# bharath5673/StrongSORT-YOLO

Hardware: NVIDIA B200
Metric: tracked frames/sec at 1080p, 100 dets/frame (higher is better)
Workload: dtype fp16 hi/lo operand pairs (~22-bit mantissa) with fp32 accumulate on tcgen05 (ReID convs, appearance cost) + fp32 (depthwise, decode, NMS) + f64 (Kalman, gating, IoU, LSAP)

## Files before the change

### strongsort-yolo_b200/csrc/reid_tc4.cu

```cuda
#include <cooperative_groups.h>

#include "ssb_common.cuh"
#include "tc_common.cuh"

namespace cg = cooperative_groups;

#ifndef SSB_DW_CHAINS
#define SSB_DW_CHAINS 3
#endif

namespace {

__host__ __device__ constexpr int cmax4(int a, int b) { return a > b ? a : b; }
__host__ __device__ constexpr int rup128_4(int a) { return (a + 127) / 128 * 128; }
__host__ __device__ constexpr int pow2cols(int c) { return c <= 32 ? 32 : c <= 64 ? 64 : c <= 128 ? 128 : c <= 256 ? 256 : 512; }

template <int CIN_, int MID_, int MIDP_, int COUT_, int H_, int W_, int R_, int NB_, bool DOWN_, int SEG_,
          int THREADS_, int MINB_, bool SPLIT_, bool PW_ = false>
struct B4 {
    static constexpr bool PW = PW_;
    static constexpr int CIN = CIN_, MID = MID_, MIDP = MIDP_, COUT = COUT_, H = H_, W = W_, R = R_, NB = NB_;
    static constexpr int SEG = SEG_, THREADS = THREADS_, MINB = MINB_;
    static constexpr bool DOWN = DOWN_, SPLIT = SPLIT_, EXCH = NB_ > 1;
    static constexpr int NWARPS = THREADS / 32, GROUPS = THREADS / 128;
    static constexpr int HW = H * W;
    static constexpr int NPX = R * W;
    static constexpr int NT = NPX / 128;
    static constexpr int MCH = MIDP / 8;
    static constexpr int CG = MID / 4;
    static constexpr int XL = W < 16 ? W : 16;
    static constexpr int CPW = 16 / XL;
    static constexpr int NCB = W / XL;
    static constexpr int NCGW = (CG / 2) / CPW;
    static constexpr int TPS = NCB * NCGW;
    static constexpr int PLANE_B = NPX * 16;
    static constexpr int MAP_HALF_B = MCH * PLANE_B, MAP_B = 2 * MAP_HALF_B;
    static constexpr int XCH = CIN / 8;
    static constexpr int XS_HALF_B = XCH * PLANE_B, XS_B = 2 * XS_HALF_B;
    static constexpr int TW = W + 2, TH = R + 2, TPX = TW * TH;
    static constexpr int T_B = CG * TPX * 16;
    static constexpr int A_B = rup128_4(cmax4(MAP_B + T_B, XS_B));
    static constexpr int LCN = 2 * MIDP;
    static constexpr int TM_C3 = NT * LCN, TM_COLS = TM_C3 + NT * COUT, TM_ALLOC = pow2cols(TM_COLS);
    static constexpr int C1W_B = CIN * MIDP * 4;
    static constexpr int DNW_HALF_B = DOWN ? CIN * COUT * 2 : 0, DNW_B = 2 * DNW_HALF_B;
    static constexpr int LCW_B = MIDP * MIDP * 4;
    static constexpr int WALL_B = C1W_B + DNW_B + 10 * LCW_B;
    static constexpr int PWW_HALF_B = COUT * COUT * 2, PWW_B = 2 * PWW_HALF_B;
    static constexpr int C3W_HALF_B = MIDP * COUT * 2, C3W_B = 2 * C3W_HALF_B;
    static constexpr int P_B1 = 0, P_LC = MIDP, P_B3 = P_LC + 100 * MIDP, P_GW1 = P_B3 + COUT;
    static constexpr int P_GB1 = P_GW1 + 2 * MIDP, P_GW2 = P_GB1 + 2, P_GB2 = P_GW2 + 2 * MIDP;
    static constexpr int NPAR = P_GB2 + MIDP;
    static constexpr int OFF_X1 = 0;
    static constexpr int OFF_A = OFF_X1 + MAP_B;
    static constexpr int OFF_W = OFF_A + A_B;
    static constexpr int OFF_C3 = OFF_W + rup128_4(WALL_B);
    static constexpr int OFF_PAR = OFF_C3 + C3W_B;
    static constexpr int OFF_GAP = OFF_PAR + rup128_4(NPAR * 4);
    static constexpr int OFF_MISC = OFF_GAP + 4 * NB * MIDP * 4;
    static constexpr int SCR_FLOATS = SEG * NCB * CG * 4;
    static constexpr int SMEM_B = OFF_MISC + 192 + (SCR_FLOATS + 2 * MIDP) * 4 + 64;
    static constexpr int SMEM_LIMIT = MINB >= 2 ? (232448 / MINB - 1024) : 232448;
    static_assert(NPX % 128 == 0, "band = whole M tiles");
    static_assert((W & (W - 1)) == 0, "W power of two");
    static_assert(NT <= 8, "per-tile barriers");
    static_assert(TM_ALLOC * MINB <= 512, "TMEM columns of the co-resident CTAs");
    static_assert(SMEM_B <= SMEM_LIMIT, "shared memory");
    static_assert(MIDP % 16 == 0 && COUT % 32 == 0 && CIN % 16 == 0 && MID % 4 == 0, "MMA shapes");
    static_assert(H % R == 0 && H / R == NB && NB <= 8, "bands / portable cluster size");
    static_assert(MID <= MIDP && COUT == 4 * MID && MIDP <= 32 && COUT * (MIDP / 8) <= THREADS, "OSBlock channel plan");
    static_assert(CG % 2 == 0 && (CG / 2) % CPW == 0 && W % XL == 0, "depthwise warp tasks");
    static_assert(SEG * TPS <= NWARPS, "depthwise warp tasks fit the CTA");
    static_assert(WALL_B + XS_B < (1 << 20), "mbarrier tx count");
    static_assert(!PW || (!DOWN && CIN == COUT && R % 2 == 0 && (PWW_B <= MAP_B || PWW_B <= WALL_B)), "fused transition");
    static constexpr int G_PAR = rup128_4(WALL_B);
    static constexpr int G_W3 = G_PAR + rup128_4(NPAR * 4);
    static constexpr int G_TOTAL = G_W3 + MIDP * COUT * 4;
};

__device__ __forceinline__ void split2(float a, float b, __half2 &h, __half2 &l) {
    h = __floats2half2_rn(a, b);
    const float2 hf = __half22float2(h);
    l = __floats2half2_rn(a - hf.x, b - hf.y);
}
__device__ __forceinline__ void split2p(float a, float b, __half2 &h, __half2 &l) {
    h = __floats2half2_rn(a, b);
    const float2 hf = __half22float2(h);
    unsigned long long v = ((unsigned long long)__float_as_uint(b) << 32) | __float_as_uint(a);
    const unsigned long long hv = ((unsigned long long)__float_as_uint(hf.y) << 32) | __float_as_uint(hf.x);
    asm("sub.rn.f32x2 %0, %0, %1;" : "+l"(v) : "l"(hv));
    l = __floats2half2_rn(__uint_as_float((uint32_t)v), __uint_as_float((uint32_t)(v >> 32)));
}
__device__ __forceinline__ void split1(float v, __half &h, __half &l) {
    h = __float2half_rn(v);
    l = __float2half_rn(v - __half2float(h));
}
__device__ __forceinline__ uint64_t dadv(uint64_t base, int units16) {
    return base + (uint64_t)(int64_t)units16;
}
__device__ __forceinline__ void mma3(uint32_t d, uint64_t ah, uint64_t al, uint64_t bh, uint64_t bl,
                                     uint32_t idesc, uint32_t acc) {
    tc::mma_f16_ss(d, ah, bh, idesc, acc);
    tc::mma_f16_ss(d, al, bh, idesc, 1);
    tc::mma_f16_ss(d, ah, bl, idesc, 1);
}
__device__ __forceinline__ void tmem_ld4_nw(uint32_t taddr, uint32_t *r) {
    asm volatile("tcgen05.ld.sync.aligned.32x32b.x4.b32 {%0, %1, %2, %3}, [%4];"
                 : "=r"(r[0]), "=r"(r[1]), "=r"(r[2]), "=r"(r[3])
                 : "r"(taddr)
                 : "memory");
}
__device__ __forceinline__ void tmem_ld8_nw(uint32_t taddr, uint32_t *r) {
    asm volatile("tcgen05.ld.sync.aligned.32x32b.x8.b32 {%0, %1, %2, %3, %4, %5, %6, %7}, [%8];"
                 : "=r"(r[0]), "=r"(r[1]), "=r"(r[2]), "=r"(r[3]), "=r"(r[4]), "=r"(r[5]), "=r"(r[6]), "=r"(r[7])
                 : "r"(taddr)
                 : "memory");
}
__device__ __forceinline__ void tmem_wait_ld() {
    asm volatile("tcgen05.wait::ld.sync.aligned;" ::: "memory");
}
__device__ __forceinline__ void cluster_arrive() { asm volatile("barrier.cluster.arrive.release.aligned;" ::: "memory"); }
__device__ __forceinline__ void cluster_wait() { asm volatile("barrier.cluster.wait.acquire.aligned;" ::: "memory"); }
__device__ __forceinline__ void cluster_arrive_relaxed() { asm volatile("barrier.cluster.arrive.relaxed.aligned;" ::: "memory"); }
__device__ __forceinline__ void st_cluster_f4(uint32_t cluster_addr, float a, float b, float c, float d) {
    asm volatile("st.shared::cluster.v4.f32 [%0], {%1, %2, %3, %4};" ::"r"(cluster_addr), "f"(a), "f"(b), "f"(c), "f"(d)
                 : "memory");
}
struct P4 { unsigned long long a, b; };
__device__ __forceinline__ P4 ldp4(const float4 *p) {
    const ulonglong2 v = *reinterpret_cast<const ulonglong2 *>(p);
    return P4{v.x, v.y};
}
__device__ __forceinline__ void fma4(P4 &o, const P4 &w, const P4 &v) {
    asm("fma.rn.f32x2 %0, %1, %2, %0;" : "+l"(o.a) : "l"(w.a), "l"(v.a));
    asm("fma.rn.f32x2 %0, %1, %2, %0;" : "+l"(o.b) : "l"(w.b), "l"(v.b));
}
__device__ __forceinline__ void mul4(P4 &o, const P4 &w, const P4 &v) {
    asm("mul.rn.f32x2 %0, %1, %2;" : "=l"(o.a) : "l"(w.a), "l"(v.a));
    asm("mul.rn.f32x2 %0, %1, %2;" : "=l"(o.b) : "l"(w.b), "l"(v.b));
}
__device__ __forceinline__ void add4(P4 &o, const P4 &v) {
    asm("add.rn.f32x2 %0, %0, %1;" : "+l"(o.a) : "l"(v.a));
    asm("add.rn.f32x2 %0, %0, %1;" : "+l"(o.b) : "l"(v.b));
}
__device__ __forceinline__ float p4x(const P4 &v) { return __uint_as_float((uint32_t)v.a); }
__device__ __forceinline__ float p4y(const P4 &v) { return __uint_as_float((uint32_t)(v.a >> 32)); }
__device__ __forceinline__ float p4z(const P4 &v) { return __uint_as_float((uint32_t)v.b); }
__device__ __forceinline__ float p4w(const P4 &v) { return __uint_as_float((uint32_t)(v.b >> 32)); }

__device__ __forceinline__ void unsplit8(const uint4 &h, const uint4 &l, float *out) {
    const __half2 *hh = reinterpret_cast<const __half2 *>(&h);
    const __half2 *ll = reinterpret_cast<const __half2 *>(&l);
#pragma unroll
    for (int j = 0; j < 4; j++) {
        const float2 a = __half22float2(hh[j]), b = __half22float2(ll[j]);
        out[2 * j] = a.x + b.x;
        out[2 * j + 1] = a.y + b.y;
    }
}

template <class C>
__global__ void __launch_bounds__(C::THREADS, C::MINB)
osblock4_kernel(const unsigned char *__restrict__ x, unsigned char *__restrict__ y,
                const unsigned char *__restrict__ wblob, int n_crops, int *__restrict__ status,
                long long *__restrict__ dbg, const unsigned char *__restrict__ pwblob) {
    extern __shared__ __align__(1024) unsigned char smem[];
    cg::cluster_group cluster = cg::this_cluster();
    const int tid = threadIdx.x, warp = tid >> 5, lane = tid & 31;
    const int quad = warp & 3, grp = warp >> 2;
    const int warp_u = __shfl_sync(0xffffffffu, warp, 0);
    const int crop = blockIdx.x / C::NB, band = blockIdx.x % C::NB;

    unsigned char *sX1 = smem + C::OFF_X1, *sP = smem + C::OFF_A;
    float4 *sT = reinterpret_cast<float4 *>(sP + C::MAP_B);
    unsigned char *sW = smem + C::OFF_W, *sC3 = smem + C::OFF_C3;
    float *sPar = reinterpret_cast<float *>(smem + C::OFF_PAR);
    float *sGap = reinterpret_cast<float *>(smem + C::OFF_GAP);
    uint64_t *bar_w = reinterpret_cast<uint64_t *>(smem + C::OFF_MISC);
    uint64_t *bar_c1 = bar_w + 1;
    uint64_t *bar_tile = bar_w + 3;
    uint64_t *bar_c3 = bar_w + 11;
    uint32_t *s_tmem = reinterpret_cast<uint32_t *>(bar_w + 16);
    float *s_scr = reinterpret_cast<float *>(smem + C::OFF_MISC + 192);

    if (warp == 0) tc::tmem_alloc(s_tmem, C::TM_ALLOC);
    if (tid == 0) {
        tc::mbar_init(bar_w, 1);
        tc::mbar_init(bar_c1, 1);
        for (int i = 0; i < 8; i++) tc::mbar_init(bar_tile + i, 1);
        tc::mbar_init(bar_c3, 1);
        tc::fence_mbar_init();
    }
    tc::fence_before_sync();
    __syncthreads();
    tc::fence_after_sync();
    const uint32_t tmem = *s_tmem;
    int dbg_n = 0;
    auto stamp = [&]() { if (dbg && blockIdx.x == 0 && tid == 0 && dbg_n < 63) dbg[1 + dbg_n++] = clock64(); };
#ifdef SSB_FINE_STAMPS
    int dbg_f = 0;
    auto fstamp = [&](int layer) {
        if (dbg && blockIdx.x == 0 && tid == 0 && (layer == 1 || layer == 2) && dbg_f < 40) { dbg[65 + dbg_f++] = clock64(); dbg[64] = dbg_f; }
    };
#else
    auto fstamp = [](int) {};
#endif
    stamp();
    bool ok = true;

    const unsigned char *xin = x + (size_t)crop * (4 * C::CIN * C::HW);
    constexpr int X_LO = 2 * C::CIN * C::HW;
    tc::pdl_launch_dependents();
    if (tid == 0) {
        constexpr int PAR_B = (C::NPAR * 4 + 15) / 16 * 16;
        tc::mbar_arrive_expect_tx(bar_w, C::WALL_B + C::XS_B + PAR_B);
        for (int o = 0; o < C::WALL_B; o += 32768) {
            const int nb = C::WALL_B - o < 32768 ? C::WALL_B - o : 32768;
            tc::bulk_g2s(sW + o, wblob + o, nb, bar_w);
        }
        tc::bulk_g2s(sPar, wblob + C::G_PAR, PAR_B, bar_w);
        tc::pdl_wait();
        for (int hl = 0; hl < 2; hl++)
            for (int ch = 0; ch < C::XCH; ch++)
                tc::bulk_g2s(sP + hl * C::XS_HALF_B + ch * C::PLANE_B,
                             xin + hl * X_LO + (size_t)ch * C::HW * 16 + (size_t)band * C::PLANE_B, C::PLANE_B, bar_w);
    }

    constexpr uint32_t IDESC_MID = tc::make_idesc_f16(128, C::MIDP);
    constexpr uint32_t IDESC_CAT = tc::make_idesc_f16(128, 2 * C::MIDP);
    constexpr uint32_t IDESC_OUT = tc::make_idesc_f16(128, C::COUT);
    const bool issuer = warp_u == (C::SEG * C::TPS < C::NWARPS ? C::SEG * C::TPS : 0);

    if (!tc::mbar_wait(bar_w, 0)) ok = false;
    tc::fence_after_sync();
    if (issuer) {
        if (tc::elect_one()) {
            const uint64_t ah0 = tc::make_smem_desc(tc::smem_u32(sP), C::PLANE_B, 128);
            const uint64_t al0 = dadv(ah0, C::XS_HALF_B / 16);
            const uint64_t bc0 = tc::make_smem_desc(tc::smem_u32(sW), 2 * C::MIDP * 16, 128);
#pragma unroll
            for (int t = 0; t < C::NT; t++) {
                const uint32_t d1 = tmem + t * C::LCN;
#pragma unroll
                for (int ks = 0; ks < C::CIN / 16; ks++) {
                    const int ka = t * 128 + ks * 2 * C::NPX;
                    tc::mma_f16_ss(d1, dadv(ah0, ka), dadv(bc0, ks * 4 * C::MIDP), IDESC_CAT, ks > 0);
                    tc::mma_f16_ss(d1, dadv(al0, ka), dadv(bc0, ks * 4 * C::MIDP), IDESC_MID, 1);
                }
                if (C::DOWN) {
                    const uint64_t dh0 = tc::make_smem_desc(tc::smem_u32(sW) + C::C1W_B, C::COUT * 16, 128);
                    const uint64_t dl0 = dadv(dh0, C::DNW_HALF_B / 16);
                    const uint32_t d2 = tmem + C::TM_C3 + t * C::COUT;
#pragma unroll
                    for (int ks = 0; ks < C::CIN / 16; ks++) {
                        const int ka = t * 128 + ks * 2 * C::NPX;
                        mma3(d2, dadv(ah0, ka), dadv(al0, ka), dadv(dh0, ks * 2 * C::COUT),
                             dadv(dl0, ks * 2 * C::COUT), IDESC_OUT, ks > 0);
                    }
                }
            }
            tc::mma_commit(bar_c1);
        }
        __syncwarp();
    }
    if (!tc::mbar_wait(bar_c1, 0)) ok = false;
    tc::fence_after_sync();
    stamp();

    for (int i = tid; i < (C::MAP_B + C::T_B) / 16; i += C::THREADS)
        reinterpret_cast<uint4 *>(sP)[i] = make_uint4(0u, 0u, 0u, 0u);
    {
        constexpr int NU1 = C::NT * C::MCH, UPT1 = (NU1 + C::GROUPS - 1) / C::GROUPS;
        uint32_t va[UPT1][8], vb[UPT1][8];
#pragma unroll
        for (int e = 0; e < UPT1; e++) {
            const int u = grp + e * C::GROUPS;
            if (u < NU1) {
                const int t = u / C::MCH, kc = u - t * C::MCH;
                const uint32_t ta = tmem + ((uint32_t)(quad * 32) << 16) + t * C::LCN + kc * 8;
                tmem_ld8_nw(ta, va[e]);
                tmem_ld8_nw(ta + C::MIDP, vb[e]);
            }
        }
        tmem_wait_ld();
#pragma unroll
        for (int e = 0; e < UPT1; e++) {
            const int u = grp + e * C::GROUPS;
            if (u < NU1) {
                const int t = u / C::MCH, kc = u - t * C::MCH;
                const int p = t * 128 + quad * 32 + lane;
                const float *bias = sPar + C::P_B1 + kc * 8;
                __align__(16) __half2 h[4];
                __align__(16) __half2 l[4];
#pragma unroll
                for (int j = 0; j < 8; j += 2) {
                    const float f0 = fmaxf(__uint_as_float(va[e][j]) + __uint_as_float(vb[e][j]) + bias[j], 0.f);
                    const float f1 = fmaxf(__uint_as_float(va[e][j + 1]) + __uint_as_float(vb[e][j + 1]) + bias[j + 1], 0.f);
                    split2(f0, f1, h[j >> 1], l[j >> 1]);
                }
                unsigned char *d_hi = sX1 + kc * C::PLANE_B + p * 16;
                *reinterpret_cast<uint4 *>(d_hi) = *reinterpret_cast<uint4 *>(h);
                *reinterpret_cast<uint4 *>(d_hi + C::MAP_HALF_B) = *reinterpret_cast<uint4 *>(l);
            }
        }
    }
    bool a_pending = false;
    if (C::EXCH) { cluster_arrive(); a_pending = true; }
    tc::fence_async_smem();
    tc::fence_before_sync();
    __syncthreads();
    tc::fence_after_sync();
    stamp();

    auto issue_pw = [&](const unsigned char *src, int layer, int t0, int t1) {
        const uint64_t ah0 = tc::make_smem_desc(tc::smem_u32(src), C::PLANE_B, 128);
        const uint64_t al0 = dadv(ah0, C::MAP_HALF_B / 16);
        const uint64_t b0 = tc::make_smem_desc(tc::smem_u32(sW) + C::C1W_B + C::DNW_B + layer * C::LCW_B,
                                               2 * C::MIDP * 16, 128);
#pragma unroll
        for (int t = 0; t < C::NT; t++) {
            if (t < t0 || t >= t1) continue;
            const uint32_t d = tmem + t * C::LCN;
            if (tc::elect_one()) {
#pragma unroll
                for (int ks = 0; ks < C::MIDP / 16; ks++) {
                    tc::mma_f16_ss(d, dadv(ah0, t * 128 + ks * 2 * C::NPX), dadv(b0, ks * 4 * C::MIDP), IDESC_CAT, ks > 0);
                    tc::mma_f16_ss(d, dadv(al0, t * 128 + ks * 2 * C::NPX), dadv(b0, ks * 4 * C::MIDP), IDESC_MID, 1);
                }
                tc::mma_commit(bar_tile + t);
            }
            __syncwarp();
        }
    };
    tc::pdl_wait();
    float w3r[8];
    {
        const float *w3 = reinterpret_cast<const float *>(wblob + C::G_W3);
        const int kc = tid / C::COUT, co = tid - kc * C::COUT;
#pragma unroll
        for (int j = 0; j < 8; j++) w3r[j] = tid < C::COUT * C::MCH ? w3[(kc * 8 + j) * C::COUT + co] : 0.f;
    }
    const int dw_par = lane & 1;
    const int dw_seg = warp / C::TPS, dw_cb = (warp % C::TPS) % C::NCB;
    const int dw_cg = (((warp % C::TPS) / C::NCB) * C::CPW + lane / (2 * C::XL)) * 2 + dw_par;
    const int dw_col = dw_cb * C::XL + (lane >> 1) % C::XL;
    const uint32_t sT_up = (C::EXCH && band > 0) ? tc::mapa_u32(sT, band - 1) : 0u;
    const uint32_t sT_dn = (C::EXCH && band < C::NB - 1) ? tc::mapa_u32(sT, band + 1) : 0u;
    int lc = 0;
    uint32_t tile_par = 0, c3_par = 0;
    bool c3_pending = false;
    if (issuer) issue_pw(sX1, 0, 0, C::NT);
    for (int s = 0; s < 4; s++) {
        for (int k = 0; k <= s; k++, lc++) {
            const bool last = (k == s);
            P4 wd[9], bs;
            {
                const float *wl = sPar + C::P_LC + lc * (10 * C::MIDP) + dw_cg * 4;
#pragma unroll
                for (int tap = 0; tap < 9; tap++) wd[tap] = ldp4(reinterpret_cast<const float4 *>(wl + tap * C::MIDP));
                bs = ldp4(reinterpret_cast<const float4 *>(wl + 9 * C::MIDP));
            }
            fstamp(lc);
            {
                constexpr int NU = C::NT * C::CG, UPT = (NU + C::GROUPS - 1) / C::GROUPS;
                uint32_t ra_[UPT][4], rb_[UPT][4];
#pragma unroll
                for (int i = 0; i < UPT; i++) {
                    const int u = grp + i * C::GROUPS;
                    if (u >= NU) continue;
                    const int t = u / C::CG, cgi = u - t * C::CG;
                    if (!tc::mbar_wait(bar_tile + t, tile_par)) ok = false;
                    tc::fence_after_sync();
                    const uint32_t ta = tmem + ((uint32_t)(quad * 32) << 16) + t * C::LCN + cgi * 4;
                    tmem_ld4_nw(ta, ra_[i]);
                    tmem_ld4_nw(ta + C::MIDP, rb_[i]);
                }
                tmem_wait_ld();
                fstamp(lc);
                if (a_pending) { cluster_wait(); a_pending = false; }
                fstamp(lc);
#pragma unroll
                for (int i = 0; i < UPT; i++) {
                    const int u = grp + i * C::GROUPS;
                    if (u >= NU) continue;
                    const int t = u / C::CG, cgi = u - t * C::CG;
                    const int p = t * 128 + quad * 32 + lane;
                    const int lr = p / C::W, col = p % C::W;
                    const float v0 = __uint_as_float(ra_[i][0]) + __uint_as_float(rb_[i][0]);
                    const float v1 = __uint_as_float(ra_[i][1]) + __uint_as_float(rb_[i][1]);
                    const float v2 = __uint_as_float(ra_[i][2]) + __uint_as_float(rb_[i][2]);
                    const float v3 = __uint_as_float(ra_[i][3]) + __uint_as_float(rb_[i][3]);
                    sT[cgi * C::TPX + (lr + 1) * C::TW + col + 1] = make_float4(v0, v1, v2, v3);
                    if (C::EXCH) {
                        if (lr == 0 && sT_up)
                            st_cluster_f4(sT_up + (uint32_t)(cgi * C::TPX + (C::R + 1) * C::TW + col + 1) * 16u, v0, v1, v2, v3);
                        if (lr == C::R - 1 && sT_dn)
                            st_cluster_f4(sT_dn + (uint32_t)(cgi * C::TPX + col + 1) * 16u, v0, v1, v2, v3);
                    }
                }
            }
            tile_par ^= 1;
            fstamp(lc);
            tc::fence_before_sync();
            if (C::EXCH) { cluster_arrive(); cluster_wait(); }
            else __syncthreads();
            tc::fence_after_sync();
            fstamp(lc);
            stamp();
            if (C::PW && lc == 9 && tid == 0) {
                unsigned char *dstw = C::PWW_B <= C::MAP_B ? sX1 : sW;
                tc::mbar_arrive_expect_tx(bar_w, C::PWW_B);
                for (int o = 0; o < C::PWW_B; o += 32768) {
                    const int nb = C::PWW_B - o < 32768 ? C::PWW_B - o : 32768;
                    tc::bulk_g2s(dstw + o, pwblob + o, nb, bar_w);
                }
            }
            if (last && s < 3 && issuer) issue_pw(sX1, lc + 1, 0, C::NT);
            if (k == 0 && c3_pending) {
                if (!tc::mbar_wait(bar_c3, c3_par)) ok = false;
                c3_par ^= 1;
                c3_pending = false;
                tc::fence_after_sync();
            }
            float4 gacc = make_float4(0.f, 0.f, 0.f, 0.f);
            auto dw_rows = [&](int ra, int rb) {
                if (rb <= ra) return;
                if (dw_seg >= C::SEG) return;
                const int r0 = ra + ((rb - ra) * dw_seg) / C::SEG, r1 = ra + ((rb - ra) * (dw_seg + 1)) / C::SEG;
                if (r0 >= r1) return;
                const float4 *Tp = sT + dw_cg * C::TPX + dw_col;
                unsigned char *dbase = sP + (dw_cg >> 1) * C::PLANE_B + dw_col * 16 + dw_par * 8;
                auto ldrow = [&](P4 *w, int trow) {
#pragma unroll
                    for (int j = 0; j < 3; j++) w[j] = ldp4(Tp + trow * C::TW + j);
                };
                auto dwrow = [&](int lr, const P4 *wa, const P4 *wb, const P4 *wc) {
#if SSB_DW_CHAINS == 3
                    P4 o = bs, o1, o2;
                    fma4(o, wd[0], wa[0]);
                    mul4(o1, wd[3], wb[0]);
                    mul4(o2, wd[6], wc[0]);
                    fma4(o, wd[1], wa[1]);
                    fma4(o1, wd[4], wb[1]);
                    fma4(o2, wd[7], wc[1]);
                    fma4(o, wd[2], wa[2]);
                    fma4(o1, wd[5], wb[2]);
                    fma4(o2, wd[8], wc[2]);
                    add4(o1, o2);
                    add4(o, o1);
#else
                    P4 o = bs;
#pragma unroll
                    for (int dx = 0; dx < 3; dx++) {
                        fma4(o, wd[dx], wa[dx]);
                        fma4(o, wd[3 + dx], wb[dx]);
                        fma4(o, wd[6 + dx], wc[dx]);
                    }
#endif
                    const float ox = fmaxf(p4x(o), 0.f), oy = fmaxf(p4y(o), 0.f);
                    const float oz = fmaxf(p4z(o), 0.f), ow = fmaxf(p4w(o), 0.f);
                    if (last) { gacc.x += ox; gacc.y += oy; gacc.z += oz; gacc.w += ow; }
                    __half2 h[2], l[2];
                    split2p(ox, oy, h[0], l[0]);
                    split2p(oz, ow, h[1], l[1]);
                    unsigned char *d = dbase + lr * (C::W * 16);
                    *reinterpret_cast<uint2 *>(d) = make_uint2(*reinterpret_cast<uint32_t *>(&h[0]), *reinterpret_cast<uint32_t *>(&h[1]));
                    *reinterpret_cast<uint2 *>(d + C::MAP_HALF_B) =
                        make_uint2(*reinterpret_cast<uint32_t *>(&l[0]), *reinterpret_cast<uint32_t *>(&l[1]));
                };
                P4 w0[3], w1[3], w2[3];
                ldrow(w0, r0);
                ldrow(w1, r0 + 1);
                for (int lr = r0; lr < r1; lr += 3) {
                    ldrow(w2, lr + 2);
                    dwrow(lr, w0, w1, w2);
                    if (lr + 1 < r1) {
                        ldrow(w0, lr + 3);
                        dwrow(lr + 1, w1, w2, w0);
                    }
                    if (lr + 2 < r1) {
                        ldrow(w1, lr + 4);
                        dwrow(lr + 2, w2, w0, w1);
                    }
                }
            };
            auto publish = [&]() {
                tc::fence_async_smem();
                tc::fence_before_sync();
                __syncthreads();
                tc::fence_after_sync();
            };
            if (!last) {
                if (C::SPLIT && C::NT >= 2) {
                    constexpr int TH_ = C::NT / 2, HR = TH_ * 128 / C::W;
                    dw_rows(0, HR);
                    publish();
                    if (issuer) issue_pw(sP, lc + 1, 0, TH_);
                    dw_rows(HR, C::R);
                    if (C::EXCH) { cluster_arrive_relaxed(); a_pending = true; }
                    publish();
                    if (issuer) issue_pw(sP, lc + 1, TH_, C::NT);
                } else {
                    dw_rows(0, C::R);
                    fstamp(lc);
                    if (C::EXCH) { cluster_arrive_relaxed(); a_pending = true; }
                    publish();
                    fstamp(lc);
                    if (issuer) issue_pw(sP, lc + 1, 0, C::NT);
                    fstamp(lc);
                }
                stamp();
                continue;
            }
            dw_rows(0, C::R);
            fstamp(lc);
            {
#pragma unroll
                for (int off = C::XL; off >= 2; off >>= 1) {
                    gacc.x += __shfl_xor_sync(0xffffffffu, gacc.x, off);
                    gacc.y += __shfl_xor_sync(0xffffffffu, gacc.y, off);
                    gacc.z += __shfl_xor_sync(0xffffffffu, gacc.z, off);
                    gacc.w += __shfl_xor_sync(0xffffffffu, gacc.w, off);
                }
                if (dw_seg < C::SEG && ((lane >> 1) % C::XL) == 0)
                    *reinterpret_cast<float4 *>(s_scr + ((dw_seg * C::NCB + dw_cb) * C::CG + dw_cg) * 4) = gacc;
            }
            publish();
            fstamp(lc);
            stamp();
            if (warp == 0 && lane < C::MIDP) {
                float tot = 0.f;
                if (lane < C::MID)
                    for (int g = 0; g < C::SEG * C::NCB; g++) tot += s_scr[(g * C::CG + (lane >> 2)) * 4 + (lane & 3)];
                float *slot = sGap + (s * C::NB + band) * C::MIDP + lane;
                if (C::NB > 1) {
#pragma unroll
                    for (int b = 0; b < C::NB; b++) tc::st_cluster_f32(tc::mapa_u32(slot, b), tot);
                } else {
                    *slot = tot;
                }
            }
            fstamp(lc);
            if (C::NB > 1) cluster.sync(); else __syncthreads();
            fstamp(lc);
            if (warp * 32 < C::COUT * C::MCH) {
                float tot = 0.f;
                if (lane < C::MIDP)
                    for (int b = 0; b < C::NB; b++) tot += sGap[(s * C::NB + b) * C::MIDP + lane];
                const float m = tot / (float)(C::H * C::W);
                float h0 = lane < C::MIDP ? m * sPar[C::P_GW1 + lane * 2 + 0] : 0.f;
                float h1 = lane < C::MIDP ? m * sPar[C::P_GW1 + lane * 2 + 1] : 0.f;
#pragma unroll
                for (int off = 16; off >= 1; off >>= 1) {
                    h0 += __shfl_xor_sync(0xffffffffu, h0, off);
                    h1 += __shfl_xor_sync(0xffffffffu, h1, off);
                }
                h0 = fmaxf(h0 + sPar[C::P_GB1 + 0], 0.f);
                h1 = fmaxf(h1 + sPar[C::P_GB1 + 1], 0.f);
                float gate = 0.f;
                if (lane < C::MIDP) {
                    float g = sPar[C::P_GB2 + lane];
                    g = fmaf(h0, sPar[C::P_GW2 + lane], g);
                    g = fmaf(h1, sPar[C::P_GW2 + C::MIDP + lane], g);
                    gate = 1.f / (1.f + expf(-g));
                }
                const int u = tid;
                const int kc = u / C::COUT;
                __align__(16) __half h[8];
                __align__(16) __half l[8];
#pragma unroll
                for (int j = 0; j < 8; j++) {
                    const float gk = __shfl_sync(0xffffffffu, gate, (kc * 8 + j) & 31);
                    split1(w3r[j] * gk, h[j], l[j]);
                }
                if (u < C::COUT * C::MCH) {
                    *reinterpret_cast<uint4 *>(sC3 + (size_t)u * 16) = *reinterpret_cast<uint4 *>(h);
                    *reinterpret_cast<uint4 *>(sC3 + C::C3W_HALF_B + (size_t)u * 16) = *reinterpret_cast<uint4 *>(l);
                }
            }
            fstamp(lc);
            tc::fence_async_smem();
            tc::fence_before_sync();
            __syncthreads();
            tc::fence_after_sync();
            if (issuer) {
                const uint64_t ah0 = tc::make_smem_desc(tc::smem_u32(sP), C::PLANE_B, 128);
                const uint64_t al0 = dadv(ah0, C::MAP_HALF_B / 16);
                const uint64_t bh0 = tc::make_smem_desc(tc::smem_u32(sC3), C::COUT * 16, 128);
                const uint64_t bl0 = dadv(bh0, C::C3W_HALF_B / 16);
                const uint32_t acc0 = (C::DOWN || s > 0) ? 1u : 0u;
                if (tc::elect_one()) {
#pragma unroll
                    for (int i = 0; i < C::NT; i++) {
                        const uint32_t d = tmem + C::TM_C3 + i * C::COUT;
#pragma unroll
                        for (int ks = 0; ks < C::MIDP / 16; ks++) {
                            const int ka = i * 128 + ks * 2 * C::NPX, kb = ks * 2 * C::COUT;
                            mma3(d, dadv(ah0, ka), dadv(al0, ka), dadv(bh0, kb), dadv(bl0, kb), IDESC_OUT,
                                 ks > 0 ? 1u : acc0);
                        }
                    }
                    tc::mma_commit(bar_c3);
                }
                __syncwarp();
            }
            c3_pending = true;
            stamp();
        }
    }

    unsigned char *yout = y + (size_t)crop * (4 * C::COUT * C::HW);
    constexpr int Y_LO = 2 * C::COUT * C::HW;
    constexpr int CCH = C::COUT / 32;
    constexpr int NUE = C::NT * CCH, UE = (NUE + C::GROUPS - 1) / C::GROUPS;
    constexpr bool PREF = !C::DOWN && UE <= 2;
    uint4 xh[PREF ? UE : 1][4], xl[PREF ? UE : 1][4];
    auto load_res = [&](int u, uint4 *h, uint4 *l) {
        const int i = u / CCH, c0 = (u - i * CCH) * 32;
        const size_t gp = (size_t)band * C::NPX + i * 128 + quad * 32 + lane;
#pragma unroll
        for (int j = 0; j < 4; j++) {
            const unsigned char *src = xin + (size_t)(c0 / 8 + j) * C::HW * 16 + gp * 16;
            h[j] = *reinterpret_cast<const uint4 *>(src);
            l[j] = *reinterpret_cast<const uint4 *>(src + X_LO);
        }
    };
    if (PREF) {
#pragma unroll
        for (int e = 0; e < UE; e++) {
            const int u = grp + e * C::GROUPS;
            if (u < NUE) load_res(u, xh[PREF ? e : 0], xl[PREF ? e : 0]);
        }
    }
    if (c3_pending) {
        if (!tc::mbar_wait(bar_c3, c3_par)) ok = false;
        c3_par ^= 1;
    }
    tc::fence_after_sync();
#pragma unroll
    for (int e = 0; e < UE; e++) {
        const int u = grp + e * C::GROUPS;
        if (u >= NUE) continue;
        const int i = u / CCH, c0 = (u - i * CCH) * 32;
        const size_t gp = (size_t)band * C::NPX + i * 128 + quad * 32 + lane;
        if (!C::DOWN && !PREF) load_res(u, xh[0], xl[0]);
        float v[32];
        tc::tmem_ld32(tmem + ((uint32_t)(quad * 32) << 16) + C::TM_C3 + i * C::COUT + c0, v);
#pragma unroll
        for (int j = 0; j < 4; j++) {
            float r[8];
            if (!C::DOWN) unsplit8(xh[PREF ? e : 0][j], xl[PREF ? e : 0][j], r);
            __align__(16) __half2 h[4];
            __align__(16) __half2 l[4];
#pragma unroll
            for (int q = 0; q < 8; q += 2) {
                float f0 = v[j * 8 + q] + sPar[C::P_B3 + c0 + j * 8 + q];
                float f1 = v[j * 8 + q + 1] + sPar[C::P_B3 + c0 + j * 8 + q + 1];
                if (!C::DOWN) { f0 += r[q]; f1 += r[q + 1]; }
                split2(fmaxf(f0, 0.f), fmaxf(f1, 0.f), h[q >> 1], l[q >> 1]);
            }
            if (!C::PW) {
                unsigned char *dst = yout + (size_t)(c0 / 8 + j) * C::HW * 16 + gp * 16;
                *reinterpret_cast<uint4 *>(dst) = *reinterpret_cast<uint4 *>(h);
                *reinterpret_cast<uint4 *>(dst + Y_LO) = *reinterpret_cast<uint4 *>(l);
            } else {
                const int p = i * 128 + quad * 32 + lane, lr = p / C::W, col = p % C::W;
                const int mrow = (((lr >> 1) * (C::W / 2) + (col >> 1)) << 2) + ((lr & 1) << 1) + (col & 1);
                unsigned char *dst = sP + (c0 / 8 + j) * C::PLANE_B + mrow * 16;
                *reinterpret_cast<uint4 *>(dst) = *reinterpret_cast<uint4 *>(h);
                *reinterpret_cast<uint4 *>(dst + C::XS_HALF_B) = *reinterpret_cast<uint4 *>(l);
            }
        }
    }
    if (C::PW) {
        tc::fence_async_smem();
        if (!tc::mbar_wait(bar_w, 1)) ok = false;
        tc::fence_before_sync();
        __syncthreads();
        tc::fence_after_sync();
        if (issuer) {
            if (tc::elect_one()) {
                const unsigned char *wsm = C::PWW_B <= C::MAP_B ? sX1 : sW;
                const uint64_t ah0 = tc::make_smem_desc(tc::smem_u32(sP), C::PLANE_B, 128);
                const uint64_t al0 = dadv(ah0, C::XS_HALF_B / 16);
                const uint64_t bh0 = tc::make_smem_desc(tc::smem_u32(wsm), C::COUT * 16, 128);
                const uint64_t bl0 = dadv(bh0, C::PWW_HALF_B / 16);
#pragma unroll
                for (int t = 0; t < C::NT; t++) {
                    const uint32_t d = tmem + C::TM_C3 + t * C::COUT;
#pragma unroll
                    for (int ks = 0; ks < C::COUT / 16; ks++) {
                        const int ka = t * 128 + ks * 2 * C::NPX, kb = ks * 2 * C::COUT;
                        mma3(d, dadv(ah0, ka), dadv(al0, ka), dadv(bh0, kb), dadv(bl0, kb), IDESC_OUT, ks > 0);
                    }
                }
                tc::mma_commit(bar_c1);
            }
            __syncwarp();
        }
        if (!tc::mbar_wait(bar_c1, 1)) ok = false;
        tc::fence_after_sync();
        constexpr int HWO = C::HW / 4;
        unsigned char *pout = y + (size_t)crop * (4 * C::COUT * HWO);
        const float *pwb = reinterpret_cast<const float *>(pwblob + C::PWW_B);
        constexpr int NU2 = C::NT * (C::COUT / 16), U2 = (NU2 + C::GROUPS - 1) / C::GROUPS;
#pragma unroll 1
        for (int e = 0; e < U2; e++) {
            const int u = grp + e * C::GROUPS;
            if (u >= NU2) continue;
            const int t = u / (C::COUT / 16), c0 = (u - t * (C::COUT / 16)) * 16;
            float v[16];
            tc::tmem_ld16(tmem + ((uint32_t)(quad * 32) << 16) + C::TM_C3 + t * C::COUT + c0, v);
            const int m = quad * 32 + lane;
#pragma unroll
            for (int j = 0; j < 16; j++) {
                float f = fmaxf(v[j] + pwb[c0 + j], 0.f);
                f += __shfl_xor_sync(0xffffffffu, f, 1);
                f += __shfl_xor_sync(0xffffffffu, f, 2);
                v[j] = f * 0.25f;
            }
            if ((m & 3) == 0) {
                const size_t gpo = (size_t)band * (C::NPX / 4) + t * 32 + (m >> 2);
#pragma unroll
                for (int j = 0; j < 2; j++) {
                    __align__(16) __half2 h[4];
                    __align__(16) __half2 l[4];
#pragma unroll
                    for (int q = 0; q < 8; q += 2) split2(v[j * 8 + q], v[j * 8 + q + 1], h[q >> 1], l[q >> 1]);
                    unsigned char *dst = pout + (size_t)(c0 / 8 + j) * HWO * 16 + gpo * 16;
                    *reinterpret_cast<uint4 *>(dst) = *reinterpret_cast<uint4 *>(h);
                    *reinterpret_cast<uint4 *>(dst + 2 * C::COUT * HWO) = *reinterpret_cast<uint4 *>(l);
                }
            }
        }
    }
    stamp();
    if (dbg && blockIdx.x == 0 && tid == 0) dbg[0] = dbg_n;
    if (!ok) { if (tid == 0) atomicExch(status, 6); }
    tc::fence_before_sync();
    if (C::NB > 1) cluster.sync(); else __syncthreads();
    if (warp == 0) tc::tmem_dealloc(tmem, C::TM_ALLOC);
    (void)n_crops;
}

#ifndef SSB_S2_R
#define SSB_S2_R 8
#endif
#ifndef SSB_DW_CHAINS
#define SSB_DW_CHAINS 3
#endif
#ifndef SSB_S2_SPLIT
#define SSB_S2_SPLIT false
#endif
#ifndef SSB_S3_R
#define SSB_S3_R 16
#endif
#ifndef SSB_S3_SPLIT
#define SSB_S3_SPLIT false
#endif
constexpr int S2_THREADS = SSB_S2_R == 8 ? 256 : 512, S2_MINB = SSB_S2_R == 8 ? 2 : 1, S2_SEG = SSB_S2_R == 8 ? 2 : 3;
using K0 = B4<16, 16, 16, 64, 64, 32, SSB_S2_R, 64 / SSB_S2_R, true, S2_SEG, S2_THREADS, S2_MINB, SSB_S2_SPLIT>;
using K1 = B4<64, 16, 16, 64, 64, 32, SSB_S2_R, 64 / SSB_S2_R, false, S2_SEG, S2_THREADS, S2_MINB, SSB_S2_SPLIT>;
using K2 = B4<64, 24, 32, 96, 32, 16, SSB_S3_R, 32 / SSB_S3_R, true, 4, 512, 1, SSB_S3_SPLIT>;
using K3 = B4<96, 24, 32, 96, 32, 16, SSB_S3_R, 32 / SSB_S3_R, false, 4, 512, 1, SSB_S3_SPLIT>;
using K1F = B4<64, 16, 16, 64, 64, 32, SSB_S2_R, 64 / SSB_S2_R, false, S2_SEG, S2_THREADS, S2_MINB, SSB_S2_SPLIT, true>;
using K3F = B4<96, 24, 32, 96, 32, 16, SSB_S3_R, 32 / SSB_S3_R, false, 4, 512, 1, SSB_S3_SPLIT, true>;
using K4 = B4<96, 32, 32, 128, 16, 8, 16, 1, true, 7, 512, 1, false>;
using K5 = B4<128, 32, 32, 128, 16, 8, 16, 1, false, 7, 512, 1, false>;

template <class C>
int launch4(const unsigned char *x, unsigned char *y, const unsigned char *w, int n, int *status, long long *dbg,
            cudaStream_t st, const unsigned char *pw = nullptr) {
    static const int key = ssb_new_key();
    if (ssb_first_on_device(key))
        SSB_CHECK_CUDA(cudaFuncSetAttribute(osblock4_kernel<C>, cudaFuncAttributeMaxDynamicSharedMemorySize, C::SMEM_B));
    cudaLaunchConfig_t cfg = {};
    cfg.gridDim = dim3(n * C::NB);
    cfg.blockDim = dim3(C::THREADS);
    cfg.dynamicSmemBytes = C::SMEM_B;
    cfg.stream = st;
    cudaLaunchAttribute at[2];
    at[0].id = cudaLaunchAttributeClusterDimension;
    at[0].val.clusterDim.x = C::NB;
    at[0].val.clusterDim.y = 1;
    at[0].val.clusterDim.z = 1;
    at[1].id = cudaLaunchAttributeProgrammaticStreamSerialization;
    at[1].val.programmaticStreamSerializationAllowed = 1;
    cfg.attrs = at;
    cfg.numAttrs = ssb_pdl_enabled() ? 2 : 1;
    SSB_CHECK_CUDA(cudaLaunchKernelEx(&cfg, osblock4_kernel<C>, x, y, w, n, status, dbg, pw));
    g_ssb_launches++;
    return 0;
}

__global__ void nhwc_to_planes_kernel(const float *__restrict__ x, unsigned char *__restrict__ y, int n, int HW, int Cc) {
    const long long total = (long long)n * HW * (Cc / 8);
    for (long long i = blockIdx.x * (long long)blockDim.x + threadIdx.x; i < total; i += (long long)gridDim.x * blockDim.x) {
        const int px = (int)(i % HW);
        const int ch = (int)((i / HW) % (Cc / 8));
        const int crop = (int)(i / ((long long)HW * (Cc / 8)));
        const float *src = x + ((size_t)crop * HW + px) * Cc + ch * 8;
        __align__(16) __half2 h[4];
        __align__(16) __half2 l[4];
#pragma unroll
        for (int j = 0; j < 4; j++) split2(src[2 * j], src[2 * j + 1], h[j], l[j]);
        unsigned char *dst = y + (size_t)crop * (4 * Cc * HW) + (size_t)ch * HW * 16 + (size_t)px * 16;
        *reinterpret_cast<uint4 *>(dst) = *reinterpret_cast<uint4 *>(h);
        *reinterpret_cast<uint4 *>(dst + (size_t)2 * Cc * HW) = *reinterpret_cast<uint4 *>(l);
    }
}
__global__ void planes_to_nhwc_kernel(const unsigned char *__restrict__ x, float *__restrict__ y, int n, int HW, int Cc) {
    const long long total = (long long)n * HW * (Cc / 8);
    for (long long i = blockIdx.x * (long long)blockDim.x + threadIdx.x; i < total; i += (long long)gridDim.x * blockDim.x) {
        const int px = (int)(i % HW);
        const int ch = (int)((i / HW) % (Cc / 8));
        const int crop = (int)(i / ((long long)HW * (Cc / 8)));
        const unsigned char *src = x + (size_t)crop * (4 * Cc * HW) + (size_t)ch * HW * 16 + (size_t)px * 16;
        const uint4 h = *reinterpret_cast<const uint4 *>(src);
        const uint4 l = *reinterpret_cast<const uint4 *>(src + (size_t)2 * Cc * HW);
        float r[8];
        unsplit8(h, l, r);
        float *dst = y + ((size_t)crop * HW + px) * Cc + ch * 8;
#pragma unroll
        for (int j = 0; j < 8; j++) dst[j] = r[j];
    }
}

}

int64_t ssb_reid_tc4_block_bytes(int b) {
    switch (b) {
        case 0: return K0::G_TOTAL;
        case 1: return K1::G_TOTAL;
        case 2: return K2::G_TOTAL;
        case 3: return K3::G_TOTAL;
        case 4: return K4::G_TOTAL;
        case 5: return K5::G_TOTAL;
    }
    return -1;
}

extern long long *g_ssb_tc_dbg;

int ssb_reid_tc4_block(int b, const void *x, void *y, const unsigned char *w, int n, int *status, cudaStream_t st) {
    long long *dbg = g_ssb_tc_dbg;
    const unsigned char *xi = (const unsigned char *)x;
    unsigned char *yo = (unsigned char *)y;
    switch (b) {
        case 0: return launch4<K0>(xi, yo, w, n, status, dbg, st);
        case 1: return launch4<K1>(xi, yo, w, n, status, dbg, st);
        case 2: return launch4<K2>(xi, yo, w, n, status, dbg, st);
        case 3: return launch4<K3>(xi, yo, w, n, status, dbg, st);
        case 4: return launch4<K4>(xi, yo, w, n, status, dbg, st);
        case 5: return launch4<K5>(xi, yo, w, n, status, dbg, st);
    }
    ssb_set_error("bad OSBlock index %d", b);
    return -1;
}

int ssb_reid_tc4_block_pw(int b, const void *x, void *y, const unsigned char *w, const unsigned char *pw, int n, int *status,
                          cudaStream_t st) {
    long long *dbg = g_ssb_tc_dbg;
    const unsigned char *xi = (const unsigned char *)x;
    unsigned char *yo = (unsigned char *)y;
    if (b == 1) return launch4<K1F>(xi, yo, w, n, status, dbg, st, pw);
    if (b == 3) return launch4<K3F>(xi, yo, w, n, status, dbg, st, pw);
    ssb_set_error("only OSBlocks 1 and 3 are followed by a transition layer (got %d)", b);
    return -1;
}

int ssb_reid_nhwc_to_planes(const float *x, void *y, int n, int hw, int c, cudaStream_t st) {
    if (n <= 0) return 0;
    const long long total = (long long)n * hw * (c / 8);
    const int blocks = (int)((total + 255) / 256 < 4096 ? (total + 255) / 256 : 4096);
    nhwc_to_planes_kernel<<<blocks, 256, 0, st>>>(x, (unsigned char *)y, n, hw, c);
    SSB_CHECK_LAUNCH();
    return 0;
}
int ssb_reid_planes_to_nhwc(const void *x, float *y, int n, int hw, int c, cudaStream_t st) {
    if (n <= 0) return 0;
    const long long total = (long long)n * hw * (c / 8);
    const int blocks = (int)((total + 255) / 256 < 4096 ? (total + 255) / 256 : 4096);
    planes_to_nhwc_kernel<<<blocks, 256, 0, st>>>((const unsigned char *)x, y, n, hw, c);
    SSB_CHECK_LAUNCH();
    return 0;
}
```

Baseline: 1995.

## Interleave OSBlock lite-conv streams with multiple wavefront slots in flight

Restructures the OSBlock kernel so the four lite-conv streams (depths 1-4) run as a wavefront schedule with WF slots in flight. Each slot has its own smem activation/halo buffer, TMEM accumulators and per-tile barriers, so several streams share each step's pointwise MMA, depthwise and cluster sync. The old strictly serial stream loop paid one barrier round per layer, and this is meant to cut those rounds and overlap tensor-core work with depthwise compute. It also moves the first-layer weights into the activation region to free shared memory, and drops the old SPLIT template option. The cost is more smem and TMEM per CTA and more complex scheduling logic, which may pressure occupancy or registers.

```diff
diff --git a/strongsort-yolo_b200/csrc/reid_tc4.cu b/strongsort-yolo_b200/csrc/reid_tc4.cu
--- a/strongsort-yolo_b200/csrc/reid_tc4.cu
+++ b/strongsort-yolo_b200/csrc/reid_tc4.cu
@@ -16,12 +16,17 @@
 __host__ __device__ constexpr int pow2cols(int c) { return c <= 32 ? 32 : c <= 64 ? 64 : c <= 128 ? 128 : c <= 256 ? 256 : 512; }
 
 template <int CIN_, int MID_, int MIDP_, int COUT_, int H_, int W_, int R_, int NB_, bool DOWN_, int SEG_,
-          int THREADS_, int MINB_, bool SPLIT_, bool PW_ = false>
+          int THREADS_, int MINB_, int WF_, bool PW_ = false>
 struct B4 {
     static constexpr bool PW = PW_;
     static constexpr int CIN = CIN_, MID = MID_, MIDP = MIDP_, COUT = COUT_, H = H_, W = W_, R = R_, NB = NB_;
     static constexpr int SEG = SEG_, THREADS = THREADS_, MINB = MINB_;
-    static constexpr bool DOWN = DOWN_, SPLIT = SPLIT_, EXCH = NB_ > 1;
+    static constexpr bool DOWN = DOWN_, EXCH = NB_ > 1;
+    static constexpr int WF = WF_;
+    __host__ __device__ static constexpr int stream_start(int s) { return s < WF ? 0 : stream_start(s - WF) + (s - WF) + 1; }
+    static constexpr int NSTEP = stream_start(3) + 4;
+    static constexpr unsigned START_BITS =
+        stream_start(0) | stream_start(1) << 4 | stream_start(2) << 8 | stream_start(3) << 12;
     static constexpr int NWARPS = THREADS / 32, GROUPS = THREADS / 128;
     static constexpr int HW = H * W;
     static constexpr int NPX = R * W;
@@ -39,13 +44,16 @@
     static constexpr int XS_HALF_B = XCH * PLANE_B, XS_B = 2 * XS_HALF_B;
     static constexpr int TW = W + 2, TH = R + 2, TPX = TW * TH;
     static constexpr int T_B = CG * TPX * 16;
-    static constexpr int A_B = rup128_4(cmax4(MAP_B + T_B, XS_B));
-    static constexpr int LCN = 2 * MIDP;
-    static constexpr int TM_C3 = NT * LCN, TM_COLS = TM_C3 + NT * COUT, TM_ALLOC = pow2cols(TM_COLS);
+    static constexpr int SLOT_B = MAP_B + T_B;
     static constexpr int C1W_B = CIN * MIDP * 4;
     static constexpr int DNW_HALF_B = DOWN ? CIN * COUT * 2 : 0, DNW_B = 2 * DNW_HALF_B;
+    static constexpr int P1W_B = C1W_B + DNW_B;
     static constexpr int LCW_B = MIDP * MIDP * 4;
-    static constexpr int WALL_B = C1W_B + DNW_B + 10 * LCW_B;
+    static constexpr int SW_B = 10 * LCW_B;
+    static constexpr int WALL_B = P1W_B + SW_B;
+    static constexpr int A_B = rup128_4(cmax4(WF * SLOT_B, XS_B + P1W_B));
+    static constexpr int LCN = 2 * MIDP;
+    static constexpr int TM_C3 = WF * NT * LCN, TM_COLS = TM_C3 + NT * COUT, TM_ALLOC = pow2cols(TM_COLS);
     static constexpr int PWW_HALF_B = COUT * COUT * 2, PWW_B = 2 * PWW_HALF_B;
     static constexpr int C3W_HALF_B = MIDP * COUT * 2, C3W_B = 2 * C3W_HALF_B;
     static constexpr int P_B1 = 0, P_LC = MIDP, P_B3 = P_LC + 100 * MIDP, P_GW1 = P_B3 + COUT;
@@ -53,17 +61,19 @@
     static constexpr int NPAR = P_GB2 + MIDP;
     static constexpr int OFF_X1 = 0;
     static constexpr int OFF_A = OFF_X1 + MAP_B;
+    static constexpr int OFF_P1W = OFF_A + XS_B;
     static constexpr int OFF_W = OFF_A + A_B;
-    static constexpr int OFF_C3 = OFF_W + rup128_4(WALL_B);
+    static constexpr int OFF_C3 = OFF_W + rup128_4(SW_B);
     static constexpr int OFF_PAR = OFF_C3 + C3W_B;
     static constexpr int OFF_GAP = OFF_PAR + rup128_4(NPAR * 4);
-    static constexpr int OFF_MISC = OFF_GAP + 4 * NB * MIDP * 4;
+    static constexpr int OFF_MISC = OFF_GAP + NB * MIDP * 4;
     static constexpr int SCR_FLOATS = SEG * NCB * CG * 4;
-    static constexpr int SMEM_B = OFF_MISC + 192 + (SCR_FLOATS + 2 * MIDP) * 4 + 64;
+    static constexpr int SMEM_B = OFF_MISC + 192 + SCR_FLOATS * 4;
     static constexpr int SMEM_LIMIT = MINB >= 2 ? (232448 / MINB - 1024) : 232448;
+    static_assert(WF >= 1 && WF <= 4, "streams in flight");
     static_assert(NPX % 128 == 0, "band = whole M tiles");
     static_assert((W & (W - 1)) == 0, "W power of two");
-    static_assert(NT <= 8, "per-tile barriers");
+    static_assert(WF * NT <= 8, "per-(slot, tile) barriers");
     static_assert(TM_ALLOC * MINB <= 512, "TMEM columns of the co-resident CTAs");
     static_assert(SMEM_B <= SMEM_LIMIT, "shared memory");
     static_assert(MIDP % 16 == 0 && COUT % 32 == 0 && CIN % 16 == 0 && MID % 4 == 0, "MMA shapes");
@@ -72,7 +82,7 @@
     static_assert(CG % 2 == 0 && (CG / 2) % CPW == 0 && W % XL == 0, "depthwise warp tasks");
     static_assert(SEG * TPS <= NWARPS, "depthwise warp tasks fit the CTA");
     static_assert(WALL_B + XS_B < (1 << 20), "mbarrier tx count");
-    static_assert(!PW || (!DOWN && CIN == COUT && R % 2 == 0 && (PWW_B <= MAP_B || PWW_B <= WALL_B)), "fused transition");
+    static_assert(!PW || (!DOWN && CIN == COUT && R % 2 == 0 && (PWW_B <= MAP_B || PWW_B <= SW_B)), "fused transition");
     static constexpr int G_PAR = rup128_4(WALL_B);
     static constexpr int G_W3 = G_PAR + rup128_4(NPAR * 4);
     static constexpr int G_TOTAL = G_W3 + MIDP * COUT * 4;
@@ -171,8 +181,7 @@
     const int warp_u = __shfl_sync(0xffffffffu, warp, 0);
     const int crop = blockIdx.x / C::NB, band = blockIdx.x % C::NB;
 
-    unsigned char *sX1 = smem + C::OFF_X1, *sP = smem + C::OFF_A;
-    float4 *sT = reinterpret_cast<float4 *>(sP + C::MAP_B);
+    unsigned char *sX1 = smem + C::OFF_X1, *sP = smem + C::OFF_A, *sP1W = smem + C::OFF_P1W;
     unsigned char *sW = smem + C::OFF_W, *sC3 = smem + C::OFF_C3;
     float *sPar = reinterpret_cast<float *>(smem + C::OFF_PAR);
     float *sGap = reinterpret_cast<float *>(smem + C::OFF_GAP);
@@ -199,8 +208,8 @@
     auto stamp = [&]() { if (dbg && blockIdx.x == 0 && tid == 0 && dbg_n < 63) dbg[1 + dbg_n++] = clock64(); };
 #ifdef SSB_FINE_STAMPS
     int dbg_f = 0;
-    auto fstamp = [&](int layer) {
-        if (dbg && blockIdx.x == 0 && tid == 0 && (layer == 1 || layer == 2) && dbg_f < 40) { dbg[65 + dbg_f++] = clock64(); dbg[64] = dbg_f; }
+    auto fstamp = [&](int step) {
+        if (dbg && blockIdx.x == 0 && tid == 0 && (step == 1 || step == 2) && dbg_f < 40) { dbg[65 + dbg_f++] = clock64(); dbg[64] = dbg_f; }
     };
 #else
     auto fstamp = [](int) {};
@@ -214,10 +223,11 @@
     if (tid == 0) {
         constexpr int PAR_B = (C::NPAR * 4 + 15) / 16 * 16;
         tc::mbar_arrive_expect_tx(bar_w, C::WALL_B + C::XS_B + PAR_B);
-        for (int o = 0; o < C::WALL_B; o += 32768) {
-            const int nb = C::WALL_B - o < 32768 ? C::WALL_B - o : 32768;
-            tc::bulk_g2s(sW + o, wblob + o, nb, bar_w);
-        }
+        auto copy = [&](unsigned char *dst, const unsigned char *src, int n) {
+            for (int o = 0; o < n; o += 32768) tc::bulk_g2s(dst + o, src + o, n - o < 32768 ? n - o : 32768, bar_w);
+        };
+        copy(sP1W, wblob, C::P1W_B);
+        copy(sW, wblob + C::P1W_B, C::SW_B);
         tc::bulk_g2s(sPar, wblob + C::G_PAR, PAR_B, bar_w);
         tc::pdl_wait();
         for (int hl = 0; hl < 2; hl++)
@@ -237,7 +247,7 @@
         if (tc::elect_one()) {
             const uint64_t ah0 = tc::make_smem_desc(tc::smem_u32(sP), C::PLANE_B, 128);
             const uint64_t al0 = dadv(ah0, C::XS_HALF_B / 16);
-            const uint64_t bc0 = tc::make_smem_desc(tc::smem_u32(sW), 2 * C::MIDP * 16, 128);
+            const uint64_t bc0 = tc::make_smem_desc(tc::smem_u32(sP1W), 2 * C::MIDP * 16, 128);
 #pragma unroll
             for (int t = 0; t < C::NT; t++) {
                 const uint32_t d1 = tmem + t * C::LCN;
@@ -248,7 +258,7 @@
                     tc::mma_f16_ss(d1, dadv(al0, ka), dadv(bc0, ks * 4 * C::MIDP), IDESC_MID, 1);
                 }
                 if (C::DOWN) {
-                    const uint64_t dh0 = tc::make_smem_desc(tc::smem_u32(sW) + C::C1W_B, C::COUT * 16, 128);
+                    const uint64_t dh0 = tc::make_smem_desc(tc::smem_u32(sP1W) + C::C1W_B, C::COUT * 16, 128);
                     const uint64_t dl0 = dadv(dh0, C::DNW_HALF_B / 16);
                     const uint32_t d2 = tmem + C::TM_C3 + t * C::COUT;
 #pragma unroll
@@ -267,7 +277,7 @@
     tc::fence_after_sync();
     stamp();
 
-    for (int i = tid; i < (C::MAP_B + C::T_B) / 16; i += C::THREADS)
+    for (int i = tid; i < C::WF * C::SLOT_B / 16; i += C::THREADS)
         reinterpret_cast<uint4 *>(sP)[i] = make_uint4(0u, 0u, 0u, 0u);
     {
         constexpr int NU1 = C::NT * C::MCH, UPT1 = (NU1 + C::GROUPS - 1) / C::GROUPS;
@@ -312,47 +322,145 @@
     tc::fence_after_sync();
     stamp();
 
-    auto issue_pw = [&](const unsigned char *src, int layer, int t0, int t1) {
+    auto slot_p = [&](int j) { return sP + j * C::SLOT_B; };
+    auto slot_t = [&](int j) { return reinterpret_cast<float4 *>(sP + j * C::SLOT_B + C::MAP_B); };
+    auto issue_pw = [&](const unsigned char *src, int layer, int j) {
         const uint64_t ah0 = tc::make_smem_desc(tc::smem_u32(src), C::PLANE_B, 128);
         const uint64_t al0 = dadv(ah0, C::MAP_HALF_B / 16);
-        const uint64_t b0 = tc::make_smem_desc(tc::smem_u32(sW) + C::C1W_B + C::DNW_B + layer * C::LCW_B,
-                                               2 * C::MIDP * 16, 128);
+        const uint64_t b0 = tc::make_smem_desc(tc::smem_u32(sW) + layer * C::LCW_B, 2 * C::MIDP * 16, 128);
 #pragma unroll
         for (int t = 0; t < C::NT; t++) {
-            if (t < t0 || t >= t1) continue;
-            const uint32_t d = tmem + t * C::LCN;
+            const uint32_t d = tmem + (j * C::NT + t) * C::LCN;
             if (tc::elect_one()) {
 #pragma unroll
                 for (int ks = 0; ks < C::MIDP / 16; ks++) {
                     tc::mma_f16_ss(d, dadv(ah0, t * 128 + ks * 2 * C::NPX), dadv(b0, ks * 4 * C::MIDP), IDESC_CAT, ks > 0);
                     tc::mma_f16_ss(d, dadv(al0, t * 128 + ks * 2 * C::NPX), dadv(b0, ks * 4 * C::MIDP), IDESC_MID, 1);
                 }
-                tc::mma_commit(bar_tile + t);
+                tc::mma_commit(bar_tile + j * C::NT + t);
             }
             __syncwarp();
         }
+    };
+    auto first_step = [](int s) { return (int)((C::START_BITS >> (4 * s)) & 15u); };
+    auto slot_stream = [&](int step, int j) {
+        for (int s = j; s < 4; s += C::WF) {
+            const int k = step - first_step(s);
+            if (k >= 0 && k <= s) return s;
+        }
+        return -1;
     };
     tc::pdl_wait();
-    float w3r[8];
-    {
-        const float *w3 = reinterpret_cast<const float *>(wblob + C::G_W3);
-        const int kc = tid / C::COUT, co = tid - kc * C::COUT;
-#pragma unroll
-        for (int j = 0; j < 8; j++) w3r[j] = tid < C::COUT * C::MCH ? w3[(kc * 8 + j) * C::COUT + co] : 0.f;
-    }
     const int dw_par = lane & 1;
     const int dw_seg = warp / C::TPS, dw_cb = (warp % C::TPS) % C::NCB;
     const int dw_cg = (((warp % C::TPS) / C::NCB) * C::CPW + lane / (2 * C::XL)) * 2 + dw_par;
     const int dw_col = dw_cb * C::XL + (lane >> 1) % C::XL;
-    const uint32_t sT_up = (C::EXCH && band > 0) ? tc::mapa_u32(sT, band - 1) : 0u;
-    const uint32_t sT_dn = (C::EXCH && band < C::NB - 1) ? tc::mapa_u32(sT, band + 1) : 0u;
-    int lc = 0;
+    const uint32_t sA_up = (C::EXCH && band > 0) ? tc::mapa_u32(sP, band - 1) : 0u;
+    const uint32_t sA_dn = (C::EXCH && band < C::NB - 1) ? tc::mapa_u32(sP, band + 1) : 0u;
     uint32_t tile_par = 0, c3_par = 0;
     bool c3_pending = false;
-    if (issuer) issue_pw(sX1, 0, 0, C::NT);
-    for (int s = 0; s < 4; s++) {
-        for (int k = 0; k <= s; k++, lc++) {
-            const bool last = (k == s);
+    if (issuer) {
+#pragma unroll
+        for (int j = 0; j < C::WF; j++) issue_pw(sX1, j * (j + 1) / 2, j);
+    }
+#pragma unroll 1
+    for (int step = 0; step < C::NSTEP; step++) {
+        uint32_t on = 0;
+        int fin = -1;
+#pragma unroll
+        for (int j = 0; j < C::WF; j++) {
+            const int s = slot_stream(step, j);
+            if (s >= 0) {
+                on |= 1u << j;
+                if (step == first_step(s) + s) fin = s;
+            }
+        }
+        fstamp(step);
+#pragma unroll 1
+        for (int j = 0; j < C::WF; j++) {
+            if (!((on >> j) & 1u)) continue;
+            constexpr int NU = C::NT * C::CG, UPT = (NU + C::GROUPS - 1) / C::GROUPS;
+            uint32_t ra_[UPT][4], rb_[UPT][4];
+#pragma unroll
+            for (int i = 0; i < UPT; i++) {
+                const int u = grp + i * C::GROUPS;
+                if (u >= NU) continue;
+                const int t = u / C::CG, cgi = u - t * C::CG;
+                if (!tc::mbar_wait(bar_tile + j * C::NT + t, (tile_par >> j) & 1u)) ok = false;
+                tc::fence_after_sync();
+                const uint32_t ta = tmem + ((uint32_t)(quad * 32) << 16) + (j * C::NT + t) * C::LCN + cgi * 4;
+                tmem_ld4_nw(ta, ra_[i]);
+                tmem_ld4_nw(ta + C::MIDP, rb_[i]);
+            }
+            tmem_wait_ld();
+            fstamp(step);
+            if (a_pending) { cluster_wait(); a_pending = false; }
+            fstamp(step);
+            float4 *sT = slot_t(j);
+            const uint32_t toff = (uint32_t)(j * C::SLOT_B + C::MAP_B);
+#pragma unroll
+            for (int i = 0; i < UPT; i++) {
+                const int u = grp + i * C::GROUPS;
+                if (u >= NU) continue;
+                const int t = u / C::CG, cgi = u - t * C::CG;
+                const int p = t * 128 + quad * 32 + lane;
+                const int lr = p / C::W, col = p % C::W;
+                const float v0 = __uint_as_float(ra_[i][0]) + __uint_as_float(rb_[i][0]);
+                const float v1 = __uint_as_float(ra_[i][1]) + __uint_as_float(rb_[i][1]);
+                const float v2 = __uint_as_float(ra_[i][2]) + __uint_as_float(rb_[i][2]);
+                const float v3 = __uint_as_float(ra_[i][3]) + __uint_as_float(rb_[i][3]);
+                sT[cgi * C::TPX + (lr + 1) * C::TW + col + 1] = make_float4(v0, v1, v2, v3);
+                if (C::EXCH) {
+                    if (lr == 0 && sA_up)
+                        st_cluster_f4(sA_up + toff + (uint32_t)(cgi * C::TPX + (C::R + 1) * C::TW + col + 1) * 16u, v0, v1, v2, v3);
+                    if (lr == C::R - 1 && sA_dn)
+                        st_cluster_f4(sA_dn + toff + (uint32_t)(cgi * C::TPX + col + 1) * 16u, v0, v1, v2, v3);
+                }
+            }
+        }
+        tile_par ^= on;
+        fstamp(step);
+        tc::fence_before_sync();
+        if (C::EXCH) { cluster_arrive(); cluster_wait(); }
+        else __syncthreads();
+        tc::fence_after_sync();
+        fstamp(step);
+        stamp();
+        if (C::PW && step == C::NSTEP - 1 && tid == 0) {
+            unsigned char *dstw = C::PWW_B <= C::MAP_B ? sX1 : sW;
+            tc::mbar_arrive_expect_tx(bar_w, C::PWW_B);
+            for (int o = 0; o < C::PWW_B; o += 32768) {
+                const int nb = C::PWW_B - o < 32768 ? C::PWW_B - o : 32768;
+                tc::bulk_g2s(dstw + o, pwblob + o, nb, bar_w);
+            }
+        }
+        if (issuer) {
+#pragma unroll
+            for (int j = 0; j < C::WF; j++) {
+                const int s = slot_stream(step + 1, j);
+                if (s >= 0 && first_step(s) == step + 1) issue_pw(sX1, s * (s + 1) / 2, j);
+            }
+        }
+        float w3r[8];
+        if (fin >= 0) {
+            const float *w3 = reinterpret_cast<const float *>(wblob + C::G_W3);
+            const int kc = tid / C::COUT, co = tid - kc * C::COUT;
+#pragma unroll
+            for (int j = 0; j < 8; j++) w3r[j] = tid < C::COUT * C::MCH ? __ldg(w3 + (kc * 8 + j) * C::COUT + co) : 0.f;
+        }
+        if (c3_pending) {
+            if (!tc::mbar_wait(bar_c3, c3_par)) ok = false;
+            c3_par ^= 1;
+            c3_pending = false;
+            tc::fence_after_sync();
+        }
+        float4 gacc = make_float4(0.f, 0.f, 0.f, 0.f);
+#pragma unroll 1
+        for (int j = 0; j < C::WF; j++) {
+            const int s = slot_stream(step, j);
+            if (s < 0 || dw_seg >= C::SEG) continue;
+            const int lc = s * (s + 1) / 2 + step - first_step(s);
+            const bool last = s == fin;
             P4 wd[9], bs;
             {
                 const float *wl = sPar + C::P_LC + lc * (10 * C::MIDP) + dw_cg * 4;
@@ -360,253 +468,182 @@
                 for (int tap = 0; tap < 9; tap++) wd[tap] = ldp4(reinterpret_cast<const float4 *>(wl + tap * C::MIDP));
                 bs = ldp4(reinterpret_cast<const float4 *>(wl + 9 * C::MIDP));
             }
-            fstamp(lc);
-            {
-                constexpr int NU = C::NT * C::CG, UPT = (NU + C::GROUPS - 1) / C::GROUPS;
-                uint32_t ra_[UPT][4], rb_[UPT][4];
-#pragma unroll
-                for (int i = 0; i < UPT; i++) {
-                    const int u = grp + i * C::GROUPS;
-                    if (u >= NU) continue;
-                    const int t = u / C::CG, cgi = u - t * C::CG;
-                    if (!tc::mbar_wait(bar_tile + t, tile_par)) ok = false;
-                    tc::fence_after_sync();
-                    const uint32_t ta = tmem + ((uint32_t)(quad * 32) << 16) + t * C::LCN + cgi * 4;
-                    tmem_ld4_nw(ta, ra_[i]);
-                    tmem_ld4_nw(ta + C::MIDP, rb_[i]);
-                }
-                tmem_wait_ld();
-                fstamp(lc);
-                if (a_pending) { cluster_wait(); a_pending = false; }
-                fstamp(lc);
-#pragma unroll
-                for (int i = 0; i < UPT; i++) {
-                    const int u = grp + i * C::GROUPS;
-                    if (u >= NU) continue;
-                    const int t = u / C::CG, cgi = u - t * C::CG;
-                    const int p = t * 128 + quad * 32 + lane;
-                    const int lr = p / C::W, col = p % C::W;
-                    const float v0 = __uint_as_float(ra_[i][0]) + __uint_as_float(rb_[i][0]);
-                    const float v1 = __uint_as_float(ra_[i][1]) + __uint_as_float(rb_[i][1]);
-                    const float v2 = __uint_as_float(ra_[i][2]) + __uint_as_float(rb_[i][2]);
-                    const float v3 = __uint_as_float(ra_[i][3]) + __uint_as_float(rb_[i][3]);
-                    sT[cgi * C::TPX + (lr + 1) * C::TW + col + 1] = make_float4(v0, v1, v2, v3);
-                    if (C::EXCH) {
-                        if (lr == 0 && sT_up)
-                            st_cluster_f4(sT_up + (uint32_t)(cgi * C::TPX + (C::R + 1) * C::TW + col + 1) * 16u, v0, v1, v2, v3);
-                        if (lr == C::R - 1 && sT_dn)
-                            st_cluster_f4(sT_dn + (uint32_t)(cgi * C::TPX + col + 1) * 16u, v0, v1, v2, v3);
-                    }
-                }
-            }
-            tile_par ^= 1;
-            fstamp(lc);
-            tc::fence_before_sync();
-            if (C::EXCH) { cluster_arrive(); cluster_wait(); }
-            else __syncthreads();
-            tc::fence_after_sync();
-            fstamp(lc);
-            stamp();
-            if (C::PW && lc == 9 && tid == 0) {
-                unsigned char *dstw = C::PWW_B <= C::MAP_B ? sX1 : sW;
-                tc::mbar_arrive_expect_tx(bar_w, C::PWW_B);
-                for (int o = 0; o < C::PWW_B; o += 32768) {
-                    const int nb = C::PWW_B - o < 32768 ? C::PWW_B - o : 32768;
-                    tc::bulk_g2s(dstw + o, pwblob + o, nb, bar_w);
-                }
-            }
-            if (last && s < 3 && issuer) issue_pw(sX1, lc + 1, 0, C::NT);
-            if (k == 0 && c3_pending) {
-                if (!tc::mbar_wait(bar_c3, c3_par)) ok = false;
-                c3_par ^= 1;
-                c3_pending = false;
-                tc::fence_after_sync();
-            }
-            float4 gacc = make_float4(0.f, 0.f, 0.f, 0.f);
-            auto dw_rows = [&](int ra, int rb) {
-                if (rb <= ra) return;
-                if (dw_seg >= C::SEG) return;
-                const int r0 = ra + ((rb - ra) * dw_seg) / C::SEG, r1 = ra + ((rb - ra) * (dw_seg + 1)) / C::SEG;
-                if (r0 >= r1) return;
-                const float4 *Tp = sT + dw_cg * C::TPX + dw_col;
-                unsigned char *dbase = sP + (dw_cg >> 1) * C::PLANE_B + dw_col * 16 + dw_par * 8;
-                auto ldrow = [&](P4 *w, int trow) {
-#pragma unroll
-                    for (int j = 0; j < 3; j++) w[j] = ldp4(Tp + trow * C::TW + j);
-                };
-                auto dwrow = [&](int lr, const P4 *wa, const P4 *wb, const P4 *wc) {
+            const int r0 = (C::R * dw_seg) / C::SEG, r1 = (C::R * (dw_seg + 1)) / C::SEG;
+            if (r0 >= r1) continue;
+            const float4 *Tp = slot_t(j) + dw_cg * C::TPX + dw_col;
+            unsigned char *dbase = slot_p(j) + (dw_cg >> 1) * C::PLANE_B + dw_col * 16 + dw_par * 8;
+            auto ldrow = [&](P4 *w, int trow) {
+#pragma unroll
+                for (int x = 0; x < 3; x++) w[x] = ldp4(Tp + trow * C::TW + x);
+            };
+            auto dwrow = [&](int lr, const P4 *wa, const P4 *wb, const P4 *wc) {
 #if SSB_DW_CHAINS == 3
-                    P4 o = bs, o1, o2;
-                    fma4(o, wd[0], wa[0]);
-                    mul4(o1, wd[3], wb[0]);
-                    mul4(o2, wd[6], wc[0]);
-                    fma4(o, wd[1], wa[1]);
-                    fma4(o1, wd[4], wb[1]);
-                    fma4(o2, wd[7], wc[1]);
-                    fma4(o, wd[2], wa[2]);
-                    fma4(o1, wd[5], wb[2]);
-                    fma4(o2, wd[8], wc[2]);
-                    add4(o1, o2);
-                    add4(o, o1);
+                P4 o = bs, o1, o2;
+                fma4(o, wd[0], wa[0]);
+                mul4(o1, wd[3], wb[0]);
+                mul4(o2, wd[6], wc[0]);
+                fma4(o, wd[1], wa[1]);
+                fma4(o1, wd[4], wb[1]);
+                fma4(o2, wd[7], wc[1]);
+                fma4(o, wd[2], wa[2]);
+                fma4(o1, wd[5], wb[2]);
+                fma4(o2, wd[8], wc[2]);
+                add4(o1, o2);
+                add4(o, o1);
 #else
-                    P4 o = bs;
-#pragma unroll
-                    for (int dx = 0; dx < 3; dx++) {
-                        fma4(o, wd[dx], wa[dx]);
-                        fma4(o, wd[3 + dx], wb[dx]);
-                        fma4(o, wd[6 + dx], wc[dx]);
-                    }
+                P4 o = bs;
+#pragma unroll
+                for (int dx = 0; dx < 3; dx++) {
+                    fma4(o, wd[dx], wa[dx]);
+                    fma4(o, wd[3 + dx], wb[dx]);
+                    fma4(o, wd[6 + dx], wc[dx]);
+                }
 #endif
-                    const float ox = fmaxf(p4x(o), 0.f), oy = fmaxf(p4y(o), 0.f);
-                    const float oz = fmaxf(p4z(o), 0.f), ow = fmaxf(p4w(o), 0.f);
-                    if (last) { gacc.x += ox; gacc.y += oy; gacc.z += oz; gacc.w += ow; }
-                    __half2 h[2], l[2];
-                    split2p(ox, oy, h[0], l[0]);
-                    split2p(oz, ow, h[1], l[1]);
-                    unsigned char *d = dbase + lr * (C::W * 16);
-                    *reinterpret_cast<uint2 *>(d) = make_uint2(*reinterpret_cast<uint32_t *>(&h[0]), *reinterpret_cast<uint32_t *>(&h[1]));
-                    *reinterpret_cast<uint2 *>(d + C::MAP_HALF_B) =
-                        make_uint2(*reinterpret_cast<uint32_t *>(&l[0]), *reinterpret_cast<uint32_t *>(&l[1]));
-                };
-                P4 w0[3], w1[3], w2[3];
-                ldrow(w0, r0);
-                ldrow(w1, r0 + 1);
-                for (int lr = r0; lr < r1; lr += 3) {
-                    ldrow(w2, lr + 2);
-                    dwrow(lr, w0, w1, w2);
-                    if (lr + 1 < r1) {
-                        ldrow(w0, lr + 3);
-                        dwrow(lr + 1, w1, w2, w0);
-                    }
-                    if (lr + 2 < r1) {
-                        ldrow(w1, lr + 4);
-                        dwrow(lr + 2, w2, w0, w1);
-                    }
-                }
+                const float ox = fmaxf(p4x(o), 0.f), oy = fmaxf(p4y(o), 0.f);
+                const float oz = fmaxf(p4z(o), 0.f), ow = fmaxf(p4w(o), 0.f);
+                if (last) { gacc.x += ox; gacc.y += oy; gacc.z += oz; gacc.w += ow; }
+                __half2 h[2], l[2];
+                split2p(ox, oy, h[0], l[0]);
+                split2p(oz, ow, h[1], l[1]);
+                unsigned char *d = dbase + lr * (C::W * 16);
+                *reinterpret_cast<uint2 *>(d) = make_uint2(*reinterpret_cast<uint32_t *>(&h[0]), *reinterpret_cast<uint32_t *>(&h[1]));
+                *reinterpret_cast<uint2 *>(d + C::MAP_HALF_B) =
+                    make_uint2(*reinterpret_cast<uint32_t *>(&l[0]), *reinterpret_cast<uint32_t *>(&l[1]));
             };
-            auto publish = [&]() {
-                tc::fence_async_smem();
-                tc::fence_before_sync();
-                __syncthreads();
-                tc::fence_after_sync();
-            };
-            if (!last) {
-                if (C::SPLIT && C::NT >= 2) {
-                    constexpr int TH_ = C::NT / 2, HR = TH_ * 128 / C::W;
-                    dw_rows(0, HR);
-                    publish();
-                    if (issuer) issue_pw(sP, lc + 1, 0, TH_);
-                    dw_rows(HR, C::R);
-                    if (C::EXCH) { cluster_arrive_relaxed(); a_pending = true; }
-                    publish();
-                    if (issuer) issue_pw(sP, lc + 1, TH_, C::NT);
-                } else {
-                    dw_rows(0, C::R);
-                    fstamp(lc);
-                    if (C::EXCH) { cluster_arrive_relaxed(); a_pending = true; }
-                    publish();
-                    fstamp(lc);
-                    if (issuer) issue_pw(sP, lc + 1, 0, C::NT);
-                    fstamp(lc);
-                }
-                stamp();
-                continue;
-            }
-            dw_rows(0, C::R);
-            fstamp(lc);
-            {
-#pragma unroll
-                for (int off = C::XL; off >= 2; off >>= 1) {
-                    gacc.x += __shfl_xor_sync(0xffffffffu, gacc.x, off);
-                    gacc.y += __shfl_xor_sync(0xffffffffu, gacc.y, off);
-                    gacc.z += __shfl_xor_sync(0xffffffffu, gacc.z, off);
-                    gacc.w += __shfl_xor_sync(0xffffffffu, gacc.w, off);
-                }
-                if (dw_seg < C::SEG && ((lane >> 1) % C::XL) == 0)
-                    *reinterpret_cast<float4 *>(s_scr + ((dw_seg * C::NCB + dw_cb) * C::CG + dw_cg) * 4) = gacc;
-            }
-            publish();
-            fstamp(lc);
-            stamp();
-            if (warp == 0 && lane < C::MIDP) {
-                float tot = 0.f;
-                if (lane < C::MID)
-                    for (int g = 0; g < C::SEG * C::NCB; g++) tot += s_scr[(g * C::CG + (lane >> 2)) * 4 + (lane & 3)];
-                float *slot = sGap + (s * C::NB + band) * C::MIDP + lane;
-                if (C::NB > 1) {
-#pragma unroll
-                    for (int b = 0; b < C::NB; b++) tc::st_cluster_f32(tc::mapa_u32(slot, b), tot);
-                } else {
-                    *slot = tot;
-                }
-            }
-            fstamp(lc);
-            if (C::NB > 1) cluster.sync(); else __syncthreads();
-            fstamp(lc);
-            if (warp * 32 < C::COUT * C::MCH) {
-                float tot = 0.f;
-                if (lane < C::MIDP)
-                    for (int b = 0; b < C::NB; b++) tot += sGap[(s * C::NB + b) * C::MIDP + lane];
-                const float m = tot / (float)(C::H * C::W);
-                float h0 = lane < C::MIDP ? m * sPar[C::P_GW1 + lane * 2 + 0] : 0.f;
-                float h1 = lane < C::MIDP ? m * sPar[C::P_GW1 + lane * 2 + 1] : 0.f;
-#pragma unroll
-                for (int off = 16; off >= 1; off >>= 1) {
-                    h0 += __shfl_xor_sync(0xffffffffu, h0, off);
-                    h1 += __shfl_xor_sync(0xffffffffu, h1, off);
-                }
-                h0 = fmaxf(h0 + sPar[C::P_GB1 + 0], 0.f);
-                h1 = fmaxf(h1 + sPar[C::P_GB1 + 1], 0.f);
-                float gate = 0.f;
-                if (lane < C::MIDP) {
-                    float g = sPar[C::P_GB2 + lane];
-                    g = fmaf(h0, sPar[C::P_GW2 + lane], g);
-                    g = fmaf(h1, sPar[C::P_GW2 + C::MIDP + lane], g);
-                    gate = 1.f / (1.f + expf(-g));
-                }
-                const int u = tid;
-                const int kc = u / C::COUT;
-                __align__(16) __half h[8];
-                __align__(16) __half l[8];
-#pragma unroll
-                for (int j = 0; j < 8; j++) {
-                    const float gk = __shfl_sync(0xffffffffu, gate, (kc * 8 + j) & 31);
-                    split1(w3r[j] * gk, h[j], l[j]);
-                }
-                if (u < C::COUT * C::MCH) {
-                    *reinterpret_cast<uint4 *>(sC3 + (size_t)u * 16) = *reinterpret_cast<uint4 *>(h);
-                    *reinterpret_cast<uint4 *>(sC3 + C::C3W_HALF_B + (size_t)u * 16) = *reinterpret_cast<uint4 *>(l);
-                }
-            }
-            fstamp(lc);
+            P4 w0[3], w1[3], w2[3];
+            ldrow(w0, r0);
+            ldrow(w1, r0 + 1);
+            for (int lr = r0; lr < r1; lr += 3) {
+                ldrow(w2, lr + 2);
+                dwrow(lr, w0, w1, w2);
+                if (lr + 1 < r1) {
+                    ldrow(w0, lr + 3);
+                    dwrow(lr + 1, w1, w2, w0);
+                }
+                if (lr + 2 < r1) {
+                    ldrow(w1, lr + 4);
+                    dwrow(lr + 2, w2, w0, w1);
+                }
+            }
+        }
+        fstamp(step);
+        auto publish = [&]() {
             tc::fence_async_smem();
             tc::fence_before_sync();
             __syncthreads();
             tc::fence_after_sync();
-            if (issuer) {
-                const uint64_t ah0 = tc::make_smem_desc(tc::smem_u32(sP), C::PLANE_B, 128);
-                const uint64_t al0 = dadv(ah0, C::MAP_HALF_B / 16);
-                const uint64_t bh0 = tc::make_smem_desc(tc::smem_u32(sC3), C::COUT * 16, 128);
-                const uint64_t bl0 = dadv(bh0, C::C3W_HALF_B / 16);
-                const uint32_t acc0 = (C::DOWN || s > 0) ? 1u : 0u;
-                if (tc::elect_one()) {
-#pragma unroll
-                    for (int i = 0; i < C::NT; i++) {
-                        const uint32_t d = tmem + C::TM_C3 + i * C::COUT;
-#pragma unroll
-                        for (int ks = 0; ks < C::MIDP / 16; ks++) {
-                            const int ka = i * 128 + ks * 2 * C::NPX, kb = ks * 2 * C::COUT;
-                            mma3(d, dadv(ah0, ka), dadv(al0, ka), dadv(bh0, kb), dadv(bl0, kb), IDESC_OUT,
-                                 ks > 0 ? 1u : acc0);
-                        }
+        };
+        auto issue_next = [&]() {
+            if (!issuer) return;
+#pragma unroll
+            for (int j = 0; j < C::WF; j++) {
+                const int s = slot_stream(step, j);
+                if (s >= 0 && s != fin) issue_pw(slot_p(j), s * (s + 1) / 2 + step - first_step(s) + 1, j);
+            }
+        };
+        if (fin < 0) {
+            if (C::EXCH) { cluster_arrive_relaxed(); a_pending = true; }
+            publish();
+            fstamp(step);
+            issue_next();
+            fstamp(step);
+            stamp();
+            continue;
+        }
+        {
+#pragma unroll
+            for (int off = C::XL; off >= 2; off >>= 1) {
+                gacc.x += __shfl_xor_sync(0xffffffffu, gacc.x, off);
+                gacc.y += __shfl_xor_sync(0xffffffffu, gacc.y, off);
+                gacc.z += __shfl_xor_sync(0xffffffffu, gacc.z, off);
+                gacc.w += __shfl_xor_sync(0xffffffffu, gacc.w, off);
+            }
+            if (dw_seg < C::SEG && ((lane >> 1) % C::XL) == 0)
+                *reinterpret_cast<float4 *>(s_scr + ((dw_seg * C::NCB + dw_cb) * C::CG + dw_cg) * 4) = gacc;
+        }
+        publish();
+        fstamp(step);
+        issue_next();
+        fstamp(step);
+        stamp();
+        if (warp == 0 && lane < C::MIDP) {
+            float tot = 0.f;
+            if (lane < C::MID)
+                for (int g = 0; g < C::SEG * C::NCB; g++) tot += s_scr[(g * C::CG + (lane >> 2)) * 4 + (lane & 3)];
+            float *slot = sGap + band * C::MIDP + lane;
+            if (C::NB > 1) {
+#pragma unroll
+                for (int b = 0; b < C::NB; b++) tc::st_cluster_f32(tc::mapa_u32(slot, b), tot);
+            } else {
+                *slot = tot;
+            }
+        }
+        fstamp(step);
+        if (C::NB > 1) cluster.sync(); else __syncthreads();
+        fstamp(step);
+        if (warp * 32 < C::COUT * C::MCH) {
+            float tot = 0.f;
+            if (lane < C::MIDP)
+                for (int b = 0; b < C::NB; b++) tot += sGap[b * C::MIDP + lane];
+            const float m = tot / (float)(C::H * C::W);
+            float h0 = lane < C::MIDP ? m * sPar[C::P_GW1 + lane * 2 + 0] : 0.f;
+            float h1 = lane < C::MIDP ? m * sPar[C::P_GW1 + lane * 2 + 1] : 0.f;
+#pragma unroll
+            for (int off = 16; off >= 1; off >>= 1) {
+                h0 += __shfl_xor_sync(0xffffffffu, h0, off);
+                h1 += __shfl_xor_sync(0xffffffffu, h1, off);
+            }
+            h0 = fmaxf(h0 + sPar[C::P_GB1 + 0], 0.f);
+            h1 = fmaxf(h1 + sPar[C::P_GB1 + 1], 0.f);
+            float gate = 0.f;
+            if (lane < C::MIDP) {
+                float g = sPar[C::P_GB2 + lane];
+                g = fmaf(h0, sPar[C::P_GW2 + lane], g);
+                g = fmaf(h1, sPar[C::P_GW2 + C::MIDP + lane], g);
+                gate = 1.f / (1.f + expf(-g));
+            }
+            const int u = tid;
+            const int kc = u / C::COUT;
+            __align__(16) __half h[8];
+            __align__(16) __half l[8];
+#pragma unroll
+            for (int j = 0; j < 8; j++) {
+                const float gk = __shfl_sync(0xffffffffu, gate, (kc * 8 + j) & 31);
+                split1(w3r[j] * gk, h[j], l[j]);
+            }
+            if (u < C::COUT * C::MCH) {
+                *reinterpret_cast<uint4 *>(sC3 + (size_t)u * 16) = *reinterpret_cast<uint4 *>(h);
+                *reinterpret_cast<uint4 *>(sC3 + C::C3W_HALF_B + (size_t)u * 16) = *reinterpret_cast<uint4 *>(l);
+            }
+        }
+        fstamp(step);
+        tc::fence_async_smem();
+        tc::fence_before_sync();
+        __syncthreads();
+        tc::fence_after_sync();
+        if (issuer) {
+            const uint64_t ah0 = tc::make_smem_desc(tc::smem_u32(slot_p(fin % C::WF)), C::PLANE_B, 128);
+            const uint64_t al0 = dadv(ah0, C::MAP_HALF_B / 16);
+            const uint64_t bh0 = tc::make_smem_desc(tc::smem_u32(sC3), C::COUT * 16, 128);
+            const uint64_t bl0 = dadv(bh0, C::C3W_HALF_B / 16);
+            const uint32_t acc0 = (C::DOWN || fin > 0) ? 1u : 0u;
+            if (tc::elect_one()) {
+#pragma unroll
+                for (int i = 0; i < C::NT; i++) {
+                    const uint32_t d = tmem + C::TM_C3 + i * C::COUT;
+#pragma unroll
+                    for (int ks = 0; ks < C::MIDP / 16; ks++) {
+                        const int ka = i * 128 + ks * 2 * C::NPX, kb = ks * 2 * C::COUT;
+                        mma3(d, dadv(ah0, ka), dadv(al0, ka), dadv(bh0, kb), dadv(bl0, kb), IDESC_OUT,
+                             ks > 0 ? 1u : acc0);
                     }
-                    tc::mma_commit(bar_c3);
-                }
-                __syncwarp();
-            }
-            c3_pending = true;
-            stamp();
-        }
+                }
+                tc::mma_commit(bar_c3);
+            }
+            __syncwarp();
+        }
+        c3_pending = true;
+        stamp();
     }
 
     unsigned char *yout = y + (size_t)crop * (4 * C::COUT * C::HW);
@@ -617,10 +654,10 @@
     uint4 xh[PREF ? UE : 1][4], xl[PREF ? UE : 1][4];
     auto load_res = [&](int u, uint4 *h, uint4 *l) {
         const int i = u / CCH, c0 = (u - i * CCH) * 32;
-        const size_t gp = (size_t)band * C::NPX + i * 128 + quad * 32 + lane;
+        const int gp = band * C::NPX + i * 128 + quad * 32 + lane;
 #pragma unroll
         for (int j = 0; j < 4; j++) {
-            const unsigned char *src = xin + (size_t)(c0 / 8 + j) * C::HW * 16 + gp * 16;
+            const unsigned char *src = xin + ((c0 / 8 + j) * C::HW + gp) * 16;
             h[j] = *reinterpret_cast<const uint4 *>(src);
             l[j] = *reinterpret_cast<const uint4 *>(src + X_LO);
         }
@@ -642,7 +679,7 @@
         const int u = grp + e * C::GROUPS;
         if (u >= NUE) continue;
         const int i = u / CCH, c0 = (u - i * CCH) * 32;
-        const size_t gp = (size_t)band * C::NPX + i * 128 + quad * 32 + lane;
+        const int gp = band * C::NPX + i * 128 + quad * 32 + lane;
         if (!C::DOWN && !PREF) load_res(u, xh[0], xl[0]);
         float v[32];
         tc::tmem_ld32(tmem + ((uint32_t)(quad * 32) << 16) + C::TM_C3 + i * C::COUT + c0, v);
@@ -660,7 +697,7 @@
                 split2(fmaxf(f0, 0.f), fmaxf(f1, 0.f), h[q >> 1], l[q >> 1]);
             }
             if (!C::PW) {
-                unsigned char *dst = yout + (size_t)(c0 / 8 + j) * C::HW * 16 + gp * 16;
+                unsigned char *dst = yout + ((c0 / 8 + j) * C::HW + gp) * 16;
                 *reinterpret_cast<uint4 *>(dst) = *reinterpret_cast<uint4 *>(h);
                 *reinterpret_cast<uint4 *>(dst + Y_LO) = *reinterpret_cast<uint4 *>(l);
             } else {
@@ -749,24 +786,19 @@
 #ifndef SSB_DW_CHAINS
 #define SSB_DW_CHAINS 3
 #endif
-#ifndef SSB_S2_SPLIT
-#define SSB_S2_SPLIT false
-#endif
 #ifndef SSB_S3_R
 #define SSB_S3_R 16
 #endif
-#ifndef SSB_S3_SPLIT
-#define SSB_S3_SPLIT false
-#endif
 constexpr int S2_THREADS = SSB_S2_R == 8 ? 256 : 512, S2_MINB = SSB_S2_R == 8 ? 2 : 1, S2_SEG = SSB_S2_R == 8 ? 2 : 3;
-using K0 = B4<16, 16, 16, 64, 64, 32, SSB_S2_R, 64 / SSB_S2_R, true, S2_SEG, S2_THREADS, S2_MINB, SSB_S2_SPLIT>;
-using K1 = B4<64, 16, 16, 64, 64, 32, SSB_S2_R, 64 / SSB_S2_R, false, S2_SEG, S2_THREADS, S2_MINB, SSB_S2_SPLIT>;
-using K2 = B4<64, 24, 32, 96, 32, 16, SSB_S3_R, 32 / SSB_S3_R, true, 4, 512, 1, SSB_S3_SPLIT>;
-using K3 = B4<96, 24, 32, 96, 32, 16, SSB_S3_R, 32 / SSB_S3_R, false, 4, 512, 1, SSB_S3_SPLIT>;
-using K1F = B4<64, 16, 16, 64, 64, 32, SSB_S2_R, 64 / SSB_S2_R, false, S2_SEG, S2_THREADS, S2_MINB, SSB_S2_SPLIT, true>;
-using K3F = B4<96, 24, 32, 96, 32, 16, SSB_S3_R, 32 / SSB_S3_R, false, 4, 512, 1, SSB_S3_SPLIT, true>;
-using K4 = B4<96, 32, 32, 128, 16, 8, 16, 1, true, 7, 512, 1, false>;
-using K5 = B4<128, 32, 32, 128, 16, 8, 16, 1, false, 7, 512, 1, false>;
+constexpr int S2_WF = 2, S3_WF = 2, S4_WF = 2;
+using K0 = B4<16, 16, 16, 64, 64, 32, SSB_S2_R, 64 / SSB_S2_R, true, S2_SEG, S2_THREADS, S2_MINB, S2_WF>;
+using K1 = B4<64, 16, 16, 64, 64, 32, SSB_S2_R, 64 / SSB_S2_R, false, S2_SEG, S2_THREADS, S2_MINB, S2_WF>;
+using K2 = B4<64, 24, 32, 96, 32, 16, SSB_S3_R, 32 / SSB_S3_R, true, 4, 512, 1, S3_WF>;
+using K3 = B4<96, 24, 32, 96, 32, 16, SSB_S3_R, 32 / SSB_S3_R, false, 4, 512, 1, S3_WF>;
+using K1F = B4<64, 16, 16, 64, 64, 32, SSB_S2_R, 64 / SSB_S2_R, false, S2_SEG, S2_THREADS, S2_MINB, S2_WF, true>;
+using K3F = B4<96, 24, 32, 96, 32, 16, SSB_S3_R, 32 / SSB_S3_R, false, 4, 512, 1, S3_WF, true>;
+using K4 = B4<96, 32, 32, 128, 16, 8, 16, 1, true, 7, 512, 1, S4_WF>;
+using K5 = B4<128, 32, 32, 128, 16, 8, 16, 1, false, 7, 512, 1, S4_WF>;
 
 template <class C>
 int launch4(const unsigned char *x, unsigned char *y, const unsigned char *w, int n, int *status, long long *dbg,
```

Result: no change. 1999, median of 6 (+0.2%).
